# georghess/neurad-studio

Hardware: NVIDIA H100
Metric: rays/sec (camera+lidar) (higher is better)
Workload: dtype f32

## Files before the change

### neurad-studio_b200/csrc/b200nerf.cu

```cuda
#include <cuda_runtime.h>

#include <cstdio>
#include <cstring>
#include <new>
#include <string>
#include <vector>

#include "../../include/b200nerf.h"
#include "nff_device.h"
#include "nff_lane.h"
#include "rgb_decoder.cuh"
#include "modules.cuh"
#include "lidar_eval.cuh"
#include "lidar_loss.cuh"
#include "image_metrics.cuh"
#include "camera_rays.h"
#include "lidar_sim.cuh"

using namespace nff;

static thread_local std::string g_err;
static int fail(int code, const std::string& msg) {
  g_err = msg;
  return code;
// ... 197 lines not shown
    int64_t patch;
    if (it < full_rounds) {
      patch = (it * gridDim.x + blockIdx.x) * kPPU + warp;
    } else {
      patch = p0 + warp + (it - full_rounds) * kPPU;
      if (patch >= p1) break;
    }
    int64_t ray;
    const bool active = lane_patch_ray(P, patch, lane_, &ray);
    const LaneRay R = lane_ray_setup<ACTORS, EDIT>(P, sc, tid, ray);
    float* col = active ? handoff + ray : sc.bins2 + tid;
    sample_ray_lane<LAYOUT, ACTORS, TRACED>(P, sc, R, tid, ray, active, col, active ? P.n_rays : (int64_t)kLaneThreads,
                                            shared_edges ? e0_tab : nullptr);
  }
}
template <int LAYOUT>
static auto sample_lane_kernel(bool actors, bool traced, bool edit) {
  if (edit) return traced ? nff_sample_lane_kernel<LAYOUT, true, true, true> : nff_sample_lane_kernel<LAYOUT, true, false, true>;
  return traced ? nff_sample_lane_kernel<LAYOUT, true, true, false>
         : actors ? nff_sample_lane_kernel<LAYOUT, true, false, false>
                  : nff_sample_lane_kernel<LAYOUT, false, false, false>;
}

template <int LAYOUT, bool EDIT>
__global__ void __launch_bounds__(kLaneThreads, kLaneCtasPerSm) nff_shade_lane_kernel(const __grid_constant__ RenderParams P,
                                                                                      float* __restrict__ scratch,
                                                                                      const float* __restrict__ handoff) {
  extern __shared__ __align__(128) unsigned char smem_shade[];
  LaneTcShared* tcs = reinterpret_cast<LaneTcShared*>(smem_shade);
  const int tid = threadIdx.x, warp = __shfl_sync(0xffffffffu, (int)(threadIdx.x >> 5), 0), group = warp >> 2;
  lane_tc_stage_weights(*tcs, P.main_mlp_nn, tid, kLaneThreads);
  tc::fence_async_smem();
  __syncthreads();
  MlpLaneTc mlp;
  mlp.t = tcs;
  mlp.panel_ = reinterpret_cast<float*>(smem_shade + kLaneTcBytes);
  mlp.status = P.status;
  mlp.bar_id = 1 + group;
  const LaneScratch sc = lane_scratch_of(scratch, blockIdx.x);
  mlp.sh_tcnn = LAYOUT;
  constexpr int kPPU = kLaneThreads / 32;
  const int64_t n_patches = lane_patches(P);
  const int64_t full_rounds = n_patches / kPPU / gridDim.x;
  const int64_t r0 = full_rounds * gridDim.x * kPPU;
  const int64_t rest_groups = (n_patches - r0 + 3) / 4;
  const int64_t g0 = rest_groups * blockIdx.x / gridDim.x, g1 = rest_groups * (blockIdx.x + 1) / gridDim.x;
  for (int64_t it = 0;; ++it) {
    int64_t patch;
    if (it < full_rounds) {
      patch = (it * gridDim.x + blockIdx.x) * kPPU + warp;
    } else {
      const int64_t gu = g0 + group + (it - full_rounds) * (kLaneThreads / 128);
      if (gu >= g1) break;
      patch = r0 + gu * 4 + (warp & 3);
    }
    int64_t ray;
    const bool active = lane_patch_ray(P, patch, tid & 31, &ray);
    const LaneRay R = lane_ray_setup<true, EDIT>(P, sc, tid, ray);
    shade_ray_lane<MlpLaneTc, LAYOUT>(P, sc, R, mlp, tid, ray, active, handoff + ray, P.n_rays);
  }
}

template <bool EDIT>
__global__ void __launch_bounds__(kLaneThreads, kLaneCtasPerSm) nff_render_lane_kernel(const __grid_constant__ RenderParams P,
                                                                          float* __restrict__ scratch) {
  extern __shared__ __align__(128) unsigned char smem_lane[];
  LaneTcShared* tcs = reinterpret_cast<LaneTcShared*>(smem_lane);
  const int tid = threadIdx.x, warp = __shfl_sync(0xffffffffu, (int)(threadIdx.x >> 5), 0), group = warp >> 2;
  lane_tc_stage_weights(*tcs, P.main_mlp_nn, tid, kLaneThreads);
  tc::fence_async_smem();
  __syncthreads();
  MlpLaneTc mlp;
  mlp.t = tcs;
  mlp.panel_ = reinterpret_cast<float*>(smem_lane + kLaneTcBytes);
  mlp.status = P.status;
  mlp.bar_id = 1 + group;
  const LaneScratch sc = lane_scratch_of(scratch, blockIdx.x);
  for (int64_t unit = blockIdx.x; unit < lane_units(P); unit += gridDim.x) {
    int64_t ray;
    const bool active = lane_unit_ray(P, unit, tid, &ray);
    render_ray_lane<MlpLaneTc, 0, EDIT>(P, sc, mlp, tid, ray, active);
  }
}
// ... 653 lines not shown
  int n = 0;
  CUDA_TRY(cudaGetDeviceCount(&n));
  REQUIRE(device_ordinal >= 0 && device_ordinal < n, "device ordinal out of range");
  DeviceGuard g(device_ordinal);
  cudaDeviceProp prop;
  CUDA_TRY(cudaGetDeviceProperties(&prop, device_ordinal));
  if (prop.major != 9 || prop.minor != 0)
    return fail(B200NERF_ERR_UNSUPPORTED, "libb200nerf is built for sm_90a only (found sm_" +
                                              std::to_string(prop.major) + std::to_string(prop.minor) + ")");
  b200nerf_ctx* c = new (std::nothrow) b200nerf_ctx();
  REQUIRE(c != nullptr, "out of host memory");
  c->device = device_ordinal;
  c->sm_count = prop.multiProcessorCount;
  CUDA_TRY(cudaFuncSetAttribute(nff_render_kernel<kRenderWarps>, cudaFuncAttributeMaxDynamicSharedMemorySize,
                                (int)((kMainMlpFloats * 4 + 15) / 16 * 16 + kRenderWarps * sizeof(WarpShared))));
  CUDA_TRY(cudaFuncSetAttribute(nff_render_tc_kernel<kRenderWarps>, cudaFuncAttributeMaxDynamicSharedMemorySize,
                                (int)(tc_smem_bytes(kRenderWarps * 32) + kRenderWarps * sizeof(WarpSharedTc))));
  CUDA_TRY(cudaMalloc((void**)&c->d_status, sizeof(int)));
  CUDA_TRY(cudaMemset(c->d_status, 0, sizeof(int)));
  for (auto k : {nff_render_lane_kernel<false>, nff_render_lane_kernel<true>})
    CUDA_TRY(cudaFuncSetAttribute(k, cudaFuncAttributeMaxDynamicSharedMemorySize, (int)lane_tc_smem_bytes()));
  c->lane_ctas = c->sm_count * (kLaneCtasPerSm > NFF_SAMPLE_CTAS ? kLaneCtasPerSm : NFF_SAMPLE_CTAS);
  CUDA_TRY(cudaMalloc((void**)&c->d_lane_scratch, sizeof(float) * lane_scratch_floats_per_cta() * c->lane_ctas));
  for (auto k : {nff_shade_lane_kernel<0, false>, nff_shade_lane_kernel<1, false>, nff_shade_lane_kernel<0, true>,
                 nff_shade_lane_kernel<1, true>})
    CUDA_TRY(cudaFuncSetAttribute(k, cudaFuncAttributeMaxDynamicSharedMemorySize, (int)lane_tc_smem_bytes()));
  for (int i = 0; i < 8; ++i) {
    CUDA_TRY(cudaFuncSetAttribute(sample_lane_kernel<0>(i & 1, i & 2, i & 4), cudaFuncAttributePreferredSharedMemoryCarveout, 0));
    CUDA_TRY(cudaFuncSetAttribute(sample_lane_kernel<1>(i & 1, i & 2, i & 4), cudaFuncAttributePreferredSharedMemoryCarveout, 0));
  }
  CUDA_TRY(cudaMalloc((void**)&c->d_minmax, 2 * sizeof(unsigned)));
  c->handoff_rays = (int64_t)1 << 21;
  CUDA_TRY(cudaMalloc((void**)&c->d_handoff, sizeof(float) * (kS2 + 1) * c->handoff_rays));
  CUDA_TRY(cudaMalloc((void**)&c->d_grad_actor_ptrs, sizeof(float*) * kModMaxActors));
  CUDA_TRY(cudaMalloc((void**)&c->d_im_minmax, sizeof(float) * 4 * kImMaxBlocks));
  CUDA_TRY(cudaMalloc((void**)&c->d_im_sums, sizeof(double) * (kImMaxBlocks + kSsimMaxTiles)));
  *out = c;
  return 0;
}

int b200nerf_destroy(b200nerf_ctx* c) {
  if (!c) return 0;
  DeviceGuard g(c->device);
  for (int i = 0; i < 3; ++i) {
    cudaFree((void*)c->d_actor_tables[i]);
    cudaFree(c->d_decoder[i]);
  }
  cudaFree(c->d_main_mlp);
  cudaFree(c->d_main_mlp_nn);
// ... 356 lines not shown
    int64_t slice = c->handoff_rays;
    if (rays->image_width > 0) {
      const int64_t band = (int64_t)rays->image_width * (kLaneThreads / 32);
      REQUIRE(band <= slice, "image_width too large for the two-stage renderer");
      slice = slice / band * band;
    }
    const int fdim = kNff + c->app.dim;
    for (int64_t start = 0; start < n_rays; start += slice) {
      const int64_t cnt = n_rays - start < slice ? n_rays - start : slice;
      RenderParams Q = P;
      Q.n_rays = cnt;
      offset_rays(Q, start, fdim);
      int64_t need = (cnt + kLaneThreads - 1) / kLaneThreads;
      if (rays->image_width > 0) {
        const int64_t W = rays->image_width, H = (cnt + W - 1) / W;
        need = ((W + 31) / 32) * ((H + kLaneThreads / 32 - 1) / (kLaneThreads / 32));
      }
      const int64_t max_a = (int64_t)c->sm_count * NFF_SAMPLE_CTAS, max_b = (int64_t)c->sm_count * kLaneCtasPerSm;
      const int64_t patches = rays->image_width > 0 ? need * (kLaneThreads / 32) : (cnt + 31) / 32, groups = (patches + 3) / 4;
      const int64_t grid_a = patches < max_a ? patches : max_a, grid_b = groups < max_b ? groups : max_b;
      const bool actors = c->actors.n_actors > 0;
      if (c->layout == 1) {
        sample_lane_kernel<1>(actors, traced, edit)<<<(int)grid_a, kLaneThreads, 0, st>>>(Q, c->d_lane_scratch, c->d_handoff);
        (edit ? nff_shade_lane_kernel<1, true> : nff_shade_lane_kernel<1, false>)<<<(int)grid_b, kLaneThreads, smem, st>>>(
            Q, c->d_lane_scratch, c->d_handoff);
      } else {
        sample_lane_kernel<0>(actors, traced, edit)<<<(int)grid_a, kLaneThreads, 0, st>>>(Q, c->d_lane_scratch, c->d_handoff);
        (edit ? nff_shade_lane_kernel<0, true> : nff_shade_lane_kernel<0, false>)<<<(int)grid_b, kLaneThreads, smem, st>>>(
            Q, c->d_lane_scratch, c->d_handoff);
      }
    }
  } else if (c->mlp_mode == 2) {
    const size_t smem = lane_tc_smem_bytes();
    int64_t need = (n_rays + kLaneThreads - 1) / kLaneThreads;
    if (rays->image_width > 0) {
      const int64_t W = rays->image_width, H = (n_rays + W - 1) / W;
      need = ((W + 31) / 32) * ((H + kLaneThreads / 32 - 1) / (kLaneThreads / 32));
    }
    int lane_blocks = (int)(need < c->lane_ctas ? need : c->lane_ctas);
    (edit ? nff_render_lane_kernel<true> : nff_render_lane_kernel<false>)<<<lane_blocks, kLaneThreads, smem, st>>>(
        P, c->d_lane_scratch);
  } else if (c->mlp_mode == 1) {
    const size_t smem = tc_smem_bytes(WARPS * 32) + WARPS * sizeof(WarpSharedTc);
    nff_render_tc_kernel<WARPS><<<blocks, WARPS * 32, smem, st>>>(P);
  } else {
    const size_t smem = (kMainMlpFloats * 4 + 15) / 16 * 16 + WARPS * sizeof(WarpShared);
    nff_render_kernel<WARPS><<<blocks, WARPS * 32, smem, st>>>(P);
  }
  CUDA_TRY(cudaGetLastError());
  if (out->intensity || out->ray_drop_logit) {
    int fdim = kNff + c->app.dim;
    lidar_decode_kernel<<<(unsigned)((n_rays + 127) / 128), 128, 0, st>>>(c->d_lidar_mlp, out->features, fdim, n_rays,
// ... 1207 lines not shown
```

### neurad-studio_b200/csrc/nff_device.h

```cpp
#pragma once
#include "nff_params.h"
#include "simt.h"

#ifndef NFF_G_PROP
#define NFF_G_PROP 1
#endif
#ifndef NFF_G_ACT
#define NFF_G_ACT 2
#endif
#ifndef NFF_ILP
#define NFF_ILP 2
#endif
#ifndef NFF_F4_UNROLL
#define NFF_F4_UNROLL 2
#endif
#ifndef NFF_FAST_RCP
#define NFF_FAST_RCP 1
#endif
#ifndef NFF_PARITY_STD
#define NFF_PARITY_STD 0
#endif
#ifndef NFF_PARITY_LERP
#define NFF_PARITY_LERP 0
#endif
// ... 314 lines not shown
#pragma unroll
  for (int d = 0; d < D; ++d) w = fmul(w, (c & (1 << d)) ? frac[d] : fsub(1.0f, frac[d]));
  return w;
}
template <int D>
NFF_D float tcnn_encode_f1_dot(const Grid& gr, int L, const float* x, float std, const float* NFF_RESTRICT dec) {
  float acc = 0.0f;
#pragma unroll 1
  for (int l = 0; l < L; ++l) {
    uint32_t idx[1 << D];
    float frac[D];
    tcnn_corners<D>(gr, l, x, idx, frac);
    float f[1 << D];
#pragma unroll
    for (int c = 0; c < (1 << D); ++c) f[c] = ldg(gr.table + idx[c]);
    float v = 0.0f;
#pragma unroll
    for (int c = 0; c < (1 << D); ++c) v = fmaf(tcnn_corner_weight<D>(c, frac), f[c], v);
    acc = fmaf(fmul(v, level_weight(gr.res[l], std)), ldg(dec + l), acc);
  }
  return acc;
}
template <int D>
NFF_D void tcnn_encode_f4(const Grid& gr, int L, const float* x, float std, float* out, int stride) {
#pragma unroll 1
  for (int l = 0; l < L; ++l) {
    uint32_t idx[1 << D];
    float frac[D];
    tcnn_corners<D>(gr, l, x, idx, frac);
    const float4* t4 = reinterpret_cast<const float4*>(gr.table);
    float4 v[1 << D];
#pragma unroll
    for (int c = 0; c < (1 << D); ++c) v[c] = ldg(t4 + idx[c]);
    float a0 = 0.0f, a1 = 0.0f, a2 = 0.0f, a3 = 0.0f;
#pragma unroll
    for (int c = 0; c < (1 << D); ++c) {
      const float w = tcnn_corner_weight<D>(c, frac);
      a0 = fmaf(w, v[c].x, a0);
      a1 = fmaf(w, v[c].y, a1);
      a2 = fmaf(w, v[c].z, a2);
      a3 = fmaf(w, v[c].w, a3);
    }
    const float lw = level_weight(gr.res[l], std);
    out[(4 * l + 0) * stride] = fmul(a0, lw);
    out[(4 * l + 1) * stride] = fmul(a1, lw);
    out[(4 * l + 2) * stride] = fmul(a2, lw);
    out[(4 * l + 3) * stride] = fmul(a3, lw);
  }
}
NFF_D void sh4_tcnn(float dx, float dy, float dz, float* c) {
  const float x = fsub(fmul(fmul(fadd(dx, 1.0f), 0.5f), 2.0f), 1.0f), y = fsub(fmul(fmul(fadd(dy, 1.0f), 0.5f), 2.0f), 1.0f),
              z = fsub(fmul(fmul(fadd(dz, 1.0f), 0.5f), 2.0f), 1.0f);
  const float xy = x * y, xz = x * z, yz = y * z, x2 = x * x, y2 = y * y, z2 = z * z;
  c[0] = 0.28209479177387814f;
  c[1] = -0.48860251190291987f * y;
  c[2] = 0.48860251190291987f * z;
  c[3] = -0.48860251190291987f * x;
  c[4] = 1.0925484305920792f * xy;
  c[5] = -1.0925484305920792f * yz;
  c[6] = 0.94617469575755997f * z2 - 0.31539156525251999f;
  c[7] = -1.0925484305920792f * xz;
  c[8] = 0.54627421529603959f * x2 - 0.54627421529603959f * y2;
  c[9] = 0.59004358992664352f * y * (-3.0f * x2 + y2);
  c[10] = 2.8906114426405538f * xy * z;
  c[11] = 0.45704579946446572f * y * (1.0f - 5.0f * z2);
  c[12] = 0.3731763325901154f * z * (5.0f * z2 - 3.0f);
// ... 589 lines not shown
```

### neurad-studio_b200/csrc/nff_lane.h

```cpp
#pragma once
#include "nff_device.h"

namespace nff {

#ifndef NFF_LANE_THREADS
#define NFF_LANE_THREADS 512
#endif
#ifndef NFF_F4_WEIGHTS
#define NFF_F4_WEIGHTS 0
#endif
constexpr int kLaneThreads = NFF_LANE_THREADS;
constexpr int kLaneCtasPerSm = 512 / kLaneThreads;
constexpr int kCandFloats = 16;
constexpr int kLaneMaxCand = 32;

struct LaneScratch {
  float* w;
  float* bins1;
  float* bins2;
  float* cand;
};
NFF_HD size_t lane_scratch_floats_per_cta() {
  return (size_t)kLaneThreads * (kS0 + (kS1 + 1) + (kS2 + 1) + kLaneMaxCand * kCandFloats);
}
// ... 107 lines not shown
  float acc;
  if (a >= 0) {
    Gauss ga = {pb[0], pb[1], pb[2], g.std};
    ga = contract(ga, fg.actor_scale);
    if (LAYOUT == 1) {
      const float x4[4] = {ga.x, ga.y, ga.z, fdiv((float)a, fg.n_actors_f)};
      acc = tcnn_encode_f1_dot<4>(fg.act, 4, x4, ga.std, fg.decoder);
    } else {
      acc = encode_f1_dot<4, NFF_G_ACT>(fg.actor_tables[a], fg.act, ga, fg.decoder);
    }
  } else {
    Gauss gs = contract(g, fg.static_scale);
    if (LAYOUT == 1) {
      const float x3[3] = {gs.x, gs.y, gs.z};
      acc = tcnn_encode_f1_dot<3>(fg.stat, 6, x3, gs.std, fg.decoder);
    } else {
      acc = encode_f1_dot<6, NFF_G_PROP>(fg.stat.table, fg.stat, gs, fg.decoder);
    }
  }
  *actor_id = a;
  return expf(acc);
}

NFF_D void encode_f4_col(const float* NFF_RESTRICT table, const Grid& gr, int L, Gauss g, float* x , int pitch) {
  const uint32_t maskb = gr.mask << 4;
#pragma unroll 2
  for (int l = 0; l < L; ++l) {
    const float res = gr.res[l];
    const CellB<4> c = grid_cell_b<4>(g.x, g.y, g.z, res);
    uint32_t r[8];
    cell_offsets_b<4>(c, maskb, r);
    const char* base = level_base(table, l, gr.T, 16);
    float4 v[8];
#pragma unroll
    for (int k = 0; k < 8; ++k) v[k] = ldg_at<float4>(base, r[k]);
    float w = level_weight(res, g.std);
    const float ix = 1.0f - c.ox, iy = 1.0f - c.oy, iz = 1.0f - c.oz;
#if NFF_F4_WEIGHTS
    const float z1 = c.oz * w, z0 = iz * w;
    const float y1z1 = c.oy * z1, y0z1 = iy * z1, y1z0 = c.oy * z0, y0z0 = iy * z0;
    const float wk[8] = {c.ox * y1z1, c.ox * y0z1, ix * y0z1, ix * y1z1, c.ox * y1z0, c.ox * y0z0, ix * y0z0, ix * y1z0};
    float a0 = wk[0] * v[0].x, a1 = wk[0] * v[0].y, a2 = wk[0] * v[0].z, a3 = wk[0] * v[0].w;
#pragma unroll
    for (int k = 1; k < 8; ++k) {
      a0 = fmaf(wk[k], v[k].x, a0);
      a1 = fmaf(wk[k], v[k].y, a1);
      a2 = fmaf(wk[k], v[k].z, a2);
      a3 = fmaf(wk[k], v[k].w, a3);
    }
    x[(4 * l + 0) * pitch] = a0;
    x[(4 * l + 1) * pitch] = a1;
    x[(4 * l + 2) * pitch] = a2;
    x[(4 * l + 3) * pitch] = a3;
#else
    float f[8];
#pragma unroll
    for (int k = 0; k < 8; ++k) f[k] = v[k].x;
    x[(4 * l + 0) * pitch] = fmul(trilerp_b<4>(f, c, ix, iy, iz), w);
#pragma unroll
// ... 70 lines not shown
      c_km1 = c_k;
      if (k <= S) {
        const float wk = w_next;
        w_next = sc.w[(size_t)(k < S ? k : S - 1) * kLaneThreads + tid];
        run += (double)fdiv(fadd(wk, pad_each), tot);
        c_k = fminf(1.0f, (float)run);
      }
    }
    const int above = k > S ? S : k;
    const float b0 = edge(k - 1), b1 = edge(above);
    float t = nan_to_num(fdiv(fsub(u, c_km1), fsub(k > S ? c_km1 : c_k, c_km1)));
    t = fminf(fmaxf(t, 0.0f), 1.0f);
    const float nb = fadd(b0, fmul(t, fsub(b1, b0)));
    io.bins_out[(size_t)i * io.bins_stride] = nb;
    if (TRACED && io.tr_inds) io.tr_inds[ray * (S_new + 1) + i] = k;
    if (TRACED && io.tr_bins_s) io.tr_bins_s[ray * (S_new + 1) + i] = nb;
    if (TRACED && io.tr_bins_e) io.tr_bins_e[ray * (S_new + 1) + i] = to_euclid(nb, s_near, s_far, sp);
  }
  return depth_acc;
}

struct MlpLaneFfma {
  static constexpr int kPitch = kLaneThreads;
  const float* w;
  float* panel_;
  int sh_tcnn = 0;
  NFF_D float* panel() const { return panel_; }
  NFF_D void run(const float* x, const float dir[3], float& sdf, float* feat, int ) const {
    float h[kHidden], go[kNff + 1], in2[kNff + kSh], h2[kHidden];
    dense<kGeoIn, kHidden, kHidden, true>(w + kOffGeoW0, w + kOffGeoB0, x, h);
    dense<kHidden, kNff + 1, kGeoOutP, false>(w + kOffGeoW1, w + kOffGeoB1, h, go);
    sdf = go[0];
#pragma unroll
    for (int i = 0; i < kNff; ++i) in2[i] = go[i + 1];
    if (sh_tcnn) sh4_tcnn(dir[0], dir[1], dir[2], in2 + kNff); else sh4(dir[0], dir[1], dir[2], in2 + kNff);
    dense<kNff + kSh, kHidden, kHidden, true>(w + kOffFeatW0, w + kOffFeatB0, in2, h);
    dense<kHidden, kHidden, kHidden, true>(w + kOffFeatW1, w + kOffFeatB1, h, h2);
    dense<kHidden, kNff, kNff, false>(w + kOffFeatW2, w + kOffFeatB2, h2, h);
#pragma unroll
    for (int i = 0; i < kNff; ++i) feat[i] = in2[i] + h[i];
  }
};

#if defined(__CUDACC__)
constexpr int kLanePanelPitch = kLaneThreads + 4;
constexpr int kLanePanelRows = kGeoIn + kSh + 1;
constexpr int kLaneTcA = 6;
constexpr float kLaneTcAScale = 64.0f, kLaneTcAUnscale = 1.0f / 64.0f;
constexpr float kLaneTcOverflow = 65520.0f;
constexpr int kLaneTcRangeStatus = 4;
struct LaneTcShared {
  __half b[2 * 32 * (32 + 32 + 48 + 32 + 32)];
  float bias[kTcLayers][32];
  float up[kTcLayers], down[kTcLayers];
  float w_sdf[32];
  float b_sdf;
  unsigned wmax[kTcLayers];
};
constexpr int kLaneTcBytes = (sizeof(LaneTcShared) + 127) / 128 * 128;
constexpr size_t lane_tc_smem_bytes() { return (size_t)kLaneTcBytes + sizeof(float) * kLanePanelRows * kLanePanelPitch; }

NFF_D void lane_tc_stage_weights(LaneTcShared& t, const float* NFF_RESTRICT nn, int tid, int nthreads) {
  if (tid < kTcLayers) t.wmax[tid] = 0u;
  __syncthreads();
#pragma unroll
  for (int l = 0; l < kTcLayers; ++l) {
    unsigned m = 0u;
    for (int i = tid; i < 32 * tc_layer_k(l); i += nthreads) m = max(m, __float_as_uint(fabsf(nn[tc_layer_w(l) + i])));
    m = __reduce_max_sync(0xffffffffu, m);
    if ((tid & 31) == 0 && m) atomicMax(&t.wmax[l], m);
  }
  __syncthreads();
#pragma unroll
  for (int l = 0; l < kTcLayers; ++l) {
    int E;
    frexpf(__uint_as_float(t.wmax[l]), &E);
    const int e = min(max(15 - E, -60), 60);
    const float up = __int_as_float((127 + e) << 23), down = __int_as_float((127 - e) << 23);
    const int K = tc_layer_k(l);
    __half* hi = t.b + tc_layer_off(l);
    tc::stage_b_tile_f16(hi, hi + 32 * K, nn + tc_layer_w(l), K, up, tid, nthreads);
    for (int i = tid; i < 32; i += nthreads) t.bias[l][i] = nn[tc_layer_b(l) + i] * up * kLaneTcAScale;
    if (tid == 0) t.up[l] = up, t.down[l] = down;
  }
  for (int i = tid; i < 32; i += nthreads) t.w_sdf[i] = nn[kNnGeoW1 + i];
  if (tid == 0) t.b_sdf = nn[kNnGeoB1];
}

struct MlpLaneTc {
  static constexpr int kPitch = kLanePanelPitch;
  const LaneTcShared* t;
  float* panel_;
  int* status;
  int bar_id;
  int sh_tcnn = 0;
  NFF_D float* panel() const { return panel_; }
  NFF_D void group_sync() const { asm volatile("bar.sync %0, 128;" ::"r"(bar_id) : "memory"); }

  NFF_D static uint32_t b_desc_lo() {
    extern __shared__ __align__(128) unsigned char nff_lane_smem[];
    return tc::smem_desc_lo(tc::smem_u32(nff_lane_smem + offsetof(LaneTcShared, b)), 128u);
  }

  template <int KS, int K, int OFF>
  NFF_D void half_mma(float* acc, const float* a) const {
    uint32_t ah[4 * KS], al[4 * KS];
    float amax = 0.0f;
#pragma unroll
    for (int i = 0; i < 4 * KS; ++i) {
      amax = fmaxf(amax, fmaxf(fabsf(a[2 * i]), fabsf(a[2 * i + 1])));
      tc::f16x2_split(a[2 * i], a[2 * i + 1], ah[i], al[i]);
    }
    if (amax >= kLaneTcOverflow && status) atomicExch(status, kLaneTcRangeStatus);
    constexpr uint32_t sbo = (uint32_t)(K / 8) * 128u;
    constexpr uint32_t hi_off = (uint32_t)OFF * 2u / 16u, lo_off = (uint32_t)(OFF + 32 * K) * 2u / 16u;
    const uint32_t b_desc = b_desc_lo();
    tc::wg_fence();
#pragma unroll
    for (int ks = 0; ks < KS; ++ks) {
      const uint32_t adv = (uint32_t)(ks * 2 * 128) / 16u;
      const uint64_t dh = tc::smem_desc_of(b_desc + hi_off + adv, sbo), dl = tc::smem_desc_of(b_desc + lo_off + adv, sbo);
      tc::wgmma_f16_m64n32(acc, ah + 4 * ks, dh);
      tc::wgmma_f16_m64n32(acc, al + 4 * ks, dh);
      tc::wgmma_f16_m64n32(acc, ah + 4 * ks, dl);
    }
    tc::wg_commit();
    tc::wg_wait<0>();
    tc::reg_fence(acc, 16);
#pragma unroll
    for (int i = 0; i < 4 * KS; ++i) asm volatile("" : "+r"(ah[i]), "+r"(al[i])::"memory");
  }
  NFF_D static void load_a(float* a, const float* p, int q, int ks0, int n) {
#pragma unroll
    for (int i = 0; i < n; ++i) {
      const float* r = p + (16 * (ks0 + i) + 2 * q) * kPitch;
      a[8 * i + 0] = r[0] * kLaneTcAScale;
      a[8 * i + 1] = r[kPitch] * kLaneTcAScale;
      a[8 * i + 2] = r[8] * kLaneTcAScale;
      a[8 * i + 3] = r[kPitch + 8] * kLaneTcAScale;
      a[8 * i + 4] = r[8 * kPitch] * kLaneTcAScale;
      a[8 * i + 5] = r[9 * kPitch] * kLaneTcAScale;
      a[8 * i + 6] = r[8 * kPitch + 8] * kLaneTcAScale;
      a[8 * i + 7] = r[9 * kPitch + 8] * kLaneTcAScale;
    }
  }
  NFF_D static void bias_init(float* acc, const float* bias, int q) {
#pragma unroll
    for (int j = 0; j < 4; ++j) {
      const float2 b = *reinterpret_cast<const float2*>(bias + 8 * j + 2 * q);
      acc[4 * j + 0] = acc[4 * j + 2] = b.x;
      acc[4 * j + 1] = acc[4 * j + 3] = b.y;
    }
  }
  NFF_D static void unscale(float* acc, float down) {
#pragma unroll
    for (int i = 0; i < 16; ++i) acc[i] *= down;
  }
  NFF_D static void relu(float* acc) {
#pragma unroll
    for (int i = 0; i < 16; ++i) acc[i] = fmaxf(acc[i], 0.0f);
  }

  NFF_D void run(const float* , const float dir[3], float& sdf, float* feat, int tid) {
    float* col = panel_ + tid;
    {
      float shv[kSh];
      if (sh_tcnn) sh4_tcnn(dir[0], dir[1], dir[2], shv); else sh4(dir[0], dir[1], dir[2], shv);
#pragma unroll
      for (int i = 0; i < kSh; ++i) col[(kGeoIn + i) * kPitch] = shv[i];
    }
    group_sync();
    const int ln = tid & 31, q = ln & 3;
    float* const fr = panel_ + (tid & ~127) + 16 * ((tid >> 5) & 3) + (ln >> 2);
#pragma unroll 1
    for (int h = 0; h < 2; ++h) {
      float* const p = fr + 64 * h;
      float a[24], acc[16];
      load_a(a, p, q, 0, 2);
      bias_init(acc, t->bias[0], q);
      half_mma<2, 32, tc_layer_off(0)>(acc, a);
      unscale(acc, t->down[0]);
      relu(acc);
      float s0 = 0.0f, s1 = 0.0f;
#pragma unroll
      for (int j = 0; j < 4; ++j) {
        const float2 w = *reinterpret_cast<const float2*>(t->w_sdf + 8 * j + 2 * q);
        s0 = fmaf(acc[4 * j + 0], w.x, fmaf(acc[4 * j + 1], w.y, s0));
        s1 = fmaf(acc[4 * j + 2], w.x, fmaf(acc[4 * j + 3], w.y, s1));
      }
      s0 += __shfl_xor_sync(0xffffffffu, s0, 1);
      s1 += __shfl_xor_sync(0xffffffffu, s1, 1);
      s0 += __shfl_xor_sync(0xffffffffu, s0, 2);
      s1 += __shfl_xor_sync(0xffffffffu, s1, 2);
      if (q == 0) {
        p[(kGeoIn + kSh) * kPitch] = s0 * kLaneTcAUnscale + t->b_sdf;
        p[(kGeoIn + kSh) * kPitch + 8] = s1 * kLaneTcAUnscale + t->b_sdf;
      }
#pragma unroll
      for (int i = 0; i < 16; ++i) a[i] = acc[i];
      bias_init(acc, t->bias[1], q);
      half_mma<2, 32, tc_layer_off(1)>(acc, a);
      unscale(acc, t->down[1]);
      __syncwarp();
#pragma unroll
      for (int j = 0; j < 4; ++j) {
        float* r = p + (8 * j + 2 * q) * kPitch;
        r[0] = acc[4 * j + 0], r[kPitch] = acc[4 * j + 1], r[8] = acc[4 * j + 2], r[kPitch + 8] = acc[4 * j + 3];
      }
#pragma unroll
      for (int i = 0; i < 16; ++i) a[i] = acc[i];
      load_a(a + 16, p, q, 2, 1);
      bias_init(acc, t->bias[2], q);
      half_mma<3, 48, tc_layer_off(2)>(acc, a);
      unscale(acc, t->down[2]);
      relu(acc);
#pragma unroll
      for (int i = 0; i < 16; ++i) a[i] = acc[i];
      bias_init(acc, t->bias[3], q);
      half_mma<2, 32, tc_layer_off(3)>(acc, a);
      unscale(acc, t->down[3]);
      relu(acc);
#pragma unroll
      for (int i = 0; i < 16; ++i) a[i] = acc[i];
      bias_init(acc, t->bias[4], q);
      const float up4 = t->up[4], out4 = t->down[4] * kLaneTcAUnscale;
#pragma unroll
      for (int j = 0; j < 4; ++j) {
        const float* r = p + (8 * j + 2 * q) * kPitch;
        acc[4 * j + 0] += r[0] * up4, acc[4 * j + 1] += r[kPitch] * up4;
        acc[4 * j + 2] += r[8] * up4, acc[4 * j + 3] += r[kPitch + 8] * up4;
      }
      half_mma<2, 32, tc_layer_off(4)>(acc, a);
#pragma unroll
      for (int j = 0; j < 4; ++j) {
        float* r = p + (8 * j + 2 * q) * kPitch;
        r[0] = acc[4 * j + 0] * out4, r[kPitch] = acc[4 * j + 1] * out4;
        r[8] = acc[4 * j + 2] * out4, r[kPitch + 8] = acc[4 * j + 3] * out4;
      }
    }
    group_sync();
#pragma unroll
    for (int i = 0; i < kNff; ++i) feat[i] = col[i * kPitch];
    sdf = col[(kGeoIn + kSh) * kPitch];
  }
};
#endif

struct LaneRay {
  float o[3], d[3];
  float area, time, s_near, s_far;
  int n_cand;
};
constexpr float kDefaultNear = 0.0f, kDefaultFar = 1.0e6f;
NFF_D void lane_spacing_bounds(const Sampling& sp, float near_, float far_, float* s_near, float* s_far) {
  *s_near = spacing_fn(near_, sp);
  *s_far = spacing_fn(fminf(far_, sp.sky_distance), sp);
}
NFF_D float lane_round0_edge(const Sampling& sp, int i) {
  float s_near, s_far;
  lane_spacing_bounds(sp, kDefaultNear, kDefaultFar, &s_near, &s_far);
// ... 28 lines not shown
  const Sampling& sp = P.samp;
#pragma unroll 1
  for (int rd = 0; rd < 2; ++rd) {
    LaneRoundIO io{};
    io.S = rd == 0 ? kS0 : kS1;
    io.S_new = rd == 0 ? kS1 : kS2;
    io.u_tab = rd == 0 ? sp.u1 : sp.u2;
    io.bins_out = rd == 0 ? sc.bins1 + tid : bins2;
    io.bins_stride = rd == 0 ? (int64_t)kLaneThreads : bins2_stride;
    if (TRACED) {
      io.tr_w = !active ? nullptr : rd == 0 ? P.trace.prop_weights_0 : P.trace.prop_weights_1;
      io.tr_aid = !active ? nullptr : rd == 0 ? P.trace.actor_id_0 : P.trace.actor_id_1;
      io.tr_bins_s = !active ? nullptr : rd == 0 ? P.trace.bins_s_1 : P.trace.bins_s_2;
      io.tr_bins_e = !active ? nullptr : rd == 0 ? P.trace.bins_e_1 : P.trace.bins_e_2;
      io.tr_inds = !active ? nullptr : rd == 0 ? P.trace.inds_1 : P.trace.inds_2;
    }
    const float prop_depth = lane_proposal_round<LAYOUT, ACTORS, TRACED>(
        P, P.fields[sp.field_of_round[rd]], sc, tid, R.n_cand, io, rd == 0 ? nullptr : sc.bins1 + tid,
        rd == 0 ? e0_tab : nullptr, R.o, R.d, R.area, R.s_near, R.s_far, ray);
    if (active) (rd == 0 ? P.out.prop_depth_0 : P.out.prop_depth_1)[ray] = prop_depth;
  }
}

template <class Mlp, int LAYOUT = 0>
NFF_D void shade_ray_lane(const RenderParams& P, const LaneScratch& sc, const LaneRay& R, Mlp& mlp, int tid, int64_t ray,
                          bool active, const float* bins2, int64_t bins2_stride) {
  const Sampling& sp = P.samp;
  const float* o = R.o;
  const float* d = R.d;
  const float area = R.area, time = R.time, s_near = R.s_near, s_far = R.s_far;
  const int n_cand = R.n_cand;

  const FieldGrids& fm = P.fields[B200NERF_FIELD_MAIN];
  float fsum[kNff];
#pragma unroll
  for (int i = 0; i < kNff; ++i) fsum[i] = 0.0f;
  double T_d = 1.0;
  float acc = 0.0f, depth = 0.0f;
  float e_prev = to_euclid(bins2[0], s_near, s_far, sp);
#pragma unroll 1
  for (int s = 0; s < kS2; ++s) {
    const float e0 = e_prev;
    float e1 = to_euclid(bins2[(size_t)(s + 1) * bins2_stride], s_near, s_far, sp);
    e_prev = e1;
    if (s == kS2 - 1) e1 = fadd(e1, fsub(sp.sky_distance, e1));
    Gauss g = sample_gaussian(o, d, area, e0, e1);
    float* col = mlp.panel() + tid;
    float dir[3] = {d[0], d[1], d[2]};
    int aid = -1;
    {
      float pb[3], M[12];
      aid = n_cand > 0 ? lane_actor_of_sample(sc, tid, n_cand, g, pb, M) : -1;
      if (aid >= 0) {
        Gauss ga = {pb[0], pb[1], pb[2], g.std};
        ga = contract(ga, fm.actor_scale);
#pragma unroll
        for (int i = 16; i < 32; ++i) col[i * Mlp::kPitch] = 0.0f;
        if (LAYOUT == 1) {
          const float x4[4] = {ga.x, ga.y, ga.z, fdiv((float)aid, fm.n_actors_f)};
          tcnn_encode_f4<4>(fm.act, 4, x4, ga.std, col, Mlp::kPitch);
        } else {
          encode_f4_col(fm.actor_tables[aid], fm.act, 4, ga, col, Mlp::kPitch);
        }
        float q0 = fadd(fadd(fmul(M[0], d[0]), fmul(M[1], d[1])), fmul(M[2], d[2]));
        float q1 = fadd(fadd(fmul(M[4], d[0]), fmul(M[5], d[1])), fmul(M[6], d[2]));
        float q2 = fadd(fadd(fmul(M[8], d[0]), fmul(M[9], d[1])), fmul(M[10], d[2]));
        float n = fadd(fsqrt(fadd(fadd(fmul(q0, q0), fmul(q1, q1)), fmul(q2, q2))), 1.0e-7f);
        dir[0] = fdiv(q0, n); dir[1] = fdiv(q1, n); dir[2] = fdiv(q2, n);
      } else {
        Gauss gs = contract(g, fm.static_scale);
        if (LAYOUT == 1) {
          const float x3[3] = {gs.x, gs.y, gs.z};
          tcnn_encode_f4<3>(fm.stat, 8, x3, gs.std, col, Mlp::kPitch);
        } else {
          encode_f4_col(fm.stat.table, fm.stat, 8, gs, col, Mlp::kPitch);
        }
      }
    }
    float x[kGeoIn];
#pragma unroll
    for (int i = 0; i < kGeoIn; ++i) x[i] = col[i * Mlp::kPitch];
    float sdf, feat[kNff];
    mlp.run(x, dir, sdf, feat, tid);
    const float alpha = frcp(fadd(1.0f, expf(fmul(sdf, P.beta))));
    float w = fmul(alpha, (float)T_d);
    T_d *= (double)fsub(1.0f, alpha);
    acc = fadd(acc, w);
    if (s < kS2 - 1) depth = fadd(depth, fmul(w, fmul(fadd(e0, e1), 0.5f)));
    if (s == kS2 - 1) w = fadd(fadd(w, 1.0f), -acc);
#pragma unroll
    for (int i = 0; i < kNff; ++i) fsum[i] = fmaf(feat[i], w, fsum[i]);
    if (active) {
      if (P.trace.sdf) P.trace.sdf[ray * kS2 + s] = sdf;
      if (P.trace.alpha) P.trace.alpha[ray * kS2 + s] = alpha;
      if (P.trace.weights) P.trace.weights[ray * kS2 + s] = w;
      if (P.trace.actor_id_main) P.trace.actor_id_main[ray * kS2 + s] = aid;
      if (P.trace.field_feature) {
#pragma unroll
        for (int i = 0; i < kNff; ++i) P.trace.field_feature[(ray * kS2 + s) * kNff + i] = feat[i];
      }
    }
  }
  const int fdim = P.nff_dim + P.app.dim;
  float app[kApp];
#pragma unroll
  for (int i = 0; i < kApp; ++i) app[i] = 0.0f;
// ... 86 lines not shown
```

### neurad-studio_b200/csrc/tc_mlp.cuh

```cuda
#pragma once
#include <cuda_fp16.h>
#include <cuda_runtime.h>
#include <stdint.h>

namespace tc {

__device__ __forceinline__ uint32_t smem_u32(const void* p) { return (uint32_t)__cvta_generic_to_shared(p); }

__device__ __forceinline__ void fence_async_smem() { asm volatile("fence.proxy.async.shared::cta;" ::: "memory"); }
__device__ __forceinline__ void wg_fence() { asm volatile("wgmma.fence.sync.aligned;" ::: "memory"); }
__device__ __forceinline__ void wg_commit() { asm volatile("wgmma.commit_group.sync.aligned;" ::: "memory"); }
template <int N>
__device__ __forceinline__ void wg_wait() { asm volatile("wgmma.wait_group.sync.aligned %0;" ::"n"(N) : "memory"); }
__device__ __forceinline__ void reg_fence(float* d, int n) {
  for (int i = 0; i < n; ++i) asm volatile("" : "+f"(d[i])::"memory");
}

__device__ __forceinline__ void mbar_init(uint64_t* bar, uint32_t count) {
  asm volatile("mbarrier.init.shared::cta.b64 [%0], %1;" ::"r"(smem_u32(bar)), "r"(count) : "memory");
  asm volatile("fence.mbarrier_init.release.cluster;" ::: "memory");
}
__device__ __forceinline__ bool mbar_wait(uint64_t* bar, uint32_t parity) {
  const uint32_t addr = smem_u32(bar);
  for (int it = 0; it < (1 << 20); ++it) {
// ... 56 lines not shown
  asm volatile("{\n\t.reg .pred p;\n\tsetp.ne.b32 p, %34, 0;\n\twgmma.mma_async.sync.aligned.m64n64k16.f32.bf16.bf16 "
               "{%0, %1, %2, %3, %4, %5, %6, %7, %8, %9, %10, %11, %12, %13, %14, %15, %16, %17, %18, %19, %20, %21, %22, %23, %24, %25, %26, %27, %28, %29, %30, %31}, %32, %33, p, 1, 1, 0, 0;\n\t}"
               : TC_D32(0)
               : "l"(a_desc), "l"(b_desc), "r"(1));
}
__device__ __forceinline__ void wgmma_bf16_m64n96(float* d, uint64_t a_desc, uint64_t b_desc) {
  asm volatile("{\n\t.reg .pred p;\n\tsetp.ne.b32 p, %50, 0;\n\twgmma.mma_async.sync.aligned.m64n96k16.f32.bf16.bf16 "
               "{%0, %1, %2, %3, %4, %5, %6, %7, %8, %9, %10, %11, %12, %13, %14, %15, %16, %17, %18, %19, %20, %21, %22, %23, %24, %25, %26, %27, %28, %29, %30, %31, %32, %33, %34, %35, %36, %37, %38, %39, %40, %41, %42, %43, %44, %45, %46, %47}, %48, %49, p, 1, 1, 0, 0;\n\t}"
               : TC_D32(0), TC_D16(32)
               : "l"(a_desc), "l"(b_desc), "r"(1));
}
__device__ __forceinline__ void wgmma_bf16_m64n128(float* d, uint64_t a_desc, uint64_t b_desc) {
  asm volatile("{\n\t.reg .pred p;\n\tsetp.ne.b32 p, %66, 0;\n\twgmma.mma_async.sync.aligned.m64n128k16.f32.bf16.bf16 "
               "{%0, %1, %2, %3, %4, %5, %6, %7, %8, %9, %10, %11, %12, %13, %14, %15, %16, %17, %18, %19, %20, %21, %22, %23, %24, %25, %26, %27, %28, %29, %30, %31, %32, %33, %34, %35, %36, %37, %38, %39, %40, %41, %42, %43, %44, %45, %46, %47, %48, %49, %50, %51, %52, %53, %54, %55, %56, %57, %58, %59, %60, %61, %62, %63}, %64, %65, p, 1, 1, 0, 0;\n\t}"
               : TC_D32(0), TC_D32(32)
               : "l"(a_desc), "l"(b_desc), "r"(1));
}
__device__ __forceinline__ void wgmma_f16_m64n32(float* d, const uint32_t* a, uint64_t b_desc) {
  asm volatile("{\n\t.reg .pred p;\n\tsetp.ne.b32 p, %21, 0;\n\twgmma.mma_async.sync.aligned.m64n32k16.f32.f16.f16 "
               "{%0, %1, %2, %3, %4, %5, %6, %7, %8, %9, %10, %11, %12, %13, %14, %15}, {%16, %17, %18, %19}, %20, p, 1, 1, 0;\n\t}"
               : TC_D16(0)
               : "r"(a[0]), "r"(a[1]), "r"(a[2]), "r"(a[3]), "l"(b_desc), "r"(1));
}
template <int N>
__device__ __forceinline__ void wgmma_tf32(float* d, const uint32_t* a, uint64_t b_desc) {
  static_assert(N == 16 || N == 32 || N == 48 || N == 64, "tf32 tile widths");
  if constexpr (N == 16) wgmma_tf32_m64n16(d, a, b_desc);
  else if constexpr (N == 32) wgmma_tf32_m64n32(d, a, b_desc);
  else if constexpr (N == 48) wgmma_tf32_m64n48(d, a, b_desc);
  else wgmma_tf32_m64n64(d, a, b_desc);
}

__host__ __device__ constexpr uint32_t b_tile_floats(int n_pad, int k_pad) { return (uint32_t)(n_pad * k_pad); }
__device__ __forceinline__ uint32_t b_elem_offset(int n, int k, int k_pad) {
  return (uint32_t)((n >> 3) * (k_pad >> 2) * 32 + (k >> 2) * 32 + (n & 7) * 4 + (k & 3));
}
__device__ __forceinline__ float tf32_hi(float x) { return __uint_as_float(__float_as_uint(x) & 0xffffe000u); }

__device__ __forceinline__ void stage_b_tile(float* hi, float* lo, const float* __restrict__ w, int n_real, int k_real, int n_pad,
                                             int k_pad, int tid, int nthreads) {
  for (int i = tid; i < n_pad * k_pad; i += nthreads) {
    int n = i / k_pad, k = i % k_pad;
    float v = (n < n_real && k < k_real) ? w[n * k_real + k] : 0.0f;
    float h = tf32_hi(v);
    uint32_t off = b_elem_offset(n, k, k_pad);
    hi[off] = h;
// ... 120 lines not shown
```

Measured before the change: 91.04 million.

## Fold activation scaling into encoders and bias into epilogue; specialize shade kernel on actors

Adds an ACTORS template parameter to the shade lane kernel so scenes without actors skip actor lookup and compute the SH direction encoding once per ray rather than per sample. The TC MLP no longer multiplies A-operands by the scale when loading. Instead the encoders write pre-scaled features, the first wgmma zero-initializes the accumulator, and bias plus unscale are fused into one FMA epilogue. Overflow detection now uses half2 max on the split values, and the up factor is dropped. These changes remove per-sample multiplies and register traffic, but they alter the numerics of range checking and bias handling.

```diff
diff --git a/neurad-studio_b200/csrc/b200nerf.cu b/neurad-studio_b200/csrc/b200nerf.cu
--- a/neurad-studio_b200/csrc/b200nerf.cu
+++ b/neurad-studio_b200/csrc/b200nerf.cu
@@ -243,7 +243,7 @@
                   : nff_sample_lane_kernel<LAYOUT, false, false, false>;
 }
 
-template <int LAYOUT, bool EDIT>
+template <int LAYOUT, bool ACTORS, bool EDIT>
 __global__ void __launch_bounds__(kLaneThreads, kLaneCtasPerSm) nff_shade_lane_kernel(const __grid_constant__ RenderParams P,
                                                                                       float* __restrict__ scratch,
                                                                                       const float* __restrict__ handoff) {
@@ -277,9 +277,15 @@
     }
     int64_t ray;
     const bool active = lane_patch_ray(P, patch, tid & 31, &ray);
-    const LaneRay R = lane_ray_setup<true, EDIT>(P, sc, tid, ray);
-    shade_ray_lane<MlpLaneTc, LAYOUT>(P, sc, R, mlp, tid, ray, active, handoff + ray, P.n_rays);
-  }
+    const LaneRay R = lane_ray_setup<ACTORS, EDIT>(P, sc, tid, ray);
+    shade_ray_lane<MlpLaneTc, LAYOUT, ACTORS>(P, sc, R, mlp, tid, ray, active, handoff + ray, P.n_rays);
+  }
+}
+template <int LAYOUT>
+static auto shade_lane_kernel(bool actors, bool edit) {
+  return edit ? nff_shade_lane_kernel<LAYOUT, true, true>
+         : actors ? nff_shade_lane_kernel<LAYOUT, true, false>
+                  : nff_shade_lane_kernel<LAYOUT, false, false>;
 }
 
 template <bool EDIT>
@@ -979,9 +985,9 @@
     CUDA_TRY(cudaFuncSetAttribute(k, cudaFuncAttributeMaxDynamicSharedMemorySize, (int)lane_tc_smem_bytes()));
   c->lane_ctas = c->sm_count * (kLaneCtasPerSm > NFF_SAMPLE_CTAS ? kLaneCtasPerSm : NFF_SAMPLE_CTAS);
   CUDA_TRY(cudaMalloc((void**)&c->d_lane_scratch, sizeof(float) * lane_scratch_floats_per_cta() * c->lane_ctas));
-  for (auto k : {nff_shade_lane_kernel<0, false>, nff_shade_lane_kernel<1, false>, nff_shade_lane_kernel<0, true>,
-                 nff_shade_lane_kernel<1, true>})
-    CUDA_TRY(cudaFuncSetAttribute(k, cudaFuncAttributeMaxDynamicSharedMemorySize, (int)lane_tc_smem_bytes()));
+  for (int i = 0; i < 4; ++i)
+    for (auto k : {shade_lane_kernel<0>(i & 1, i & 2), shade_lane_kernel<1>(i & 1, i & 2)})
+      CUDA_TRY(cudaFuncSetAttribute(k, cudaFuncAttributeMaxDynamicSharedMemorySize, (int)lane_tc_smem_bytes()));
   for (int i = 0; i < 8; ++i) {
     CUDA_TRY(cudaFuncSetAttribute(sample_lane_kernel<0>(i & 1, i & 2, i & 4), cudaFuncAttributePreferredSharedMemoryCarveout, 0));
     CUDA_TRY(cudaFuncSetAttribute(sample_lane_kernel<1>(i & 1, i & 2, i & 4), cudaFuncAttributePreferredSharedMemoryCarveout, 0));
@@ -1384,12 +1390,10 @@
       const bool actors = c->actors.n_actors > 0;
       if (c->layout == 1) {
         sample_lane_kernel<1>(actors, traced, edit)<<<(int)grid_a, kLaneThreads, 0, st>>>(Q, c->d_lane_scratch, c->d_handoff);
-        (edit ? nff_shade_lane_kernel<1, true> : nff_shade_lane_kernel<1, false>)<<<(int)grid_b, kLaneThreads, smem, st>>>(
-            Q, c->d_lane_scratch, c->d_handoff);
+        shade_lane_kernel<1>(actors, edit)<<<(int)grid_b, kLaneThreads, smem, st>>>(Q, c->d_lane_scratch, c->d_handoff);
       } else {
         sample_lane_kernel<0>(actors, traced, edit)<<<(int)grid_a, kLaneThreads, 0, st>>>(Q, c->d_lane_scratch, c->d_handoff);
-        (edit ? nff_shade_lane_kernel<0, true> : nff_shade_lane_kernel<0, false>)<<<(int)grid_b, kLaneThreads, smem, st>>>(
-            Q, c->d_lane_scratch, c->d_handoff);
+        shade_lane_kernel<0>(actors, edit)<<<(int)grid_b, kLaneThreads, smem, st>>>(Q, c->d_lane_scratch, c->d_handoff);
       }
     }
   } else if (c->mlp_mode == 2) {
diff --git a/neurad-studio_b200/csrc/nff_device.h b/neurad-studio_b200/csrc/nff_device.h
--- a/neurad-studio_b200/csrc/nff_device.h
+++ b/neurad-studio_b200/csrc/nff_device.h
@@ -360,7 +360,7 @@
   return acc;
 }
 template <int D>
-NFF_D void tcnn_encode_f4(const Grid& gr, int L, const float* x, float std, float* out, int stride) {
+NFF_D void tcnn_encode_f4(const Grid& gr, int L, const float* x, float std, float* out, int stride, float scale) {
 #pragma unroll 1
   for (int l = 0; l < L; ++l) {
     uint32_t idx[1 << D];
@@ -379,7 +379,7 @@
       a2 = fmaf(w, v[c].z, a2);
       a3 = fmaf(w, v[c].w, a3);
     }
-    const float lw = level_weight(gr.res[l], std);
+    const float lw = fmul(level_weight(gr.res[l], std), scale);
     out[(4 * l + 0) * stride] = fmul(a0, lw);
     out[(4 * l + 1) * stride] = fmul(a1, lw);
     out[(4 * l + 2) * stride] = fmul(a2, lw);
diff --git a/neurad-studio_b200/csrc/nff_lane.h b/neurad-studio_b200/csrc/nff_lane.h
--- a/neurad-studio_b200/csrc/nff_lane.h
+++ b/neurad-studio_b200/csrc/nff_lane.h
@@ -153,7 +153,8 @@
   return expf(acc);
 }
 
-NFF_D void encode_f4_col(const float* NFF_RESTRICT table, const Grid& gr, int L, Gauss g, float* x , int pitch) {
+NFF_D void encode_f4_col(const float* NFF_RESTRICT table, const Grid& gr, int L, Gauss g, float* x , int pitch,
+                         float scale) {
   const uint32_t maskb = gr.mask << 4;
 #pragma unroll 2
   for (int l = 0; l < L; ++l) {
@@ -165,7 +166,7 @@
     float4 v[8];
 #pragma unroll
     for (int k = 0; k < 8; ++k) v[k] = ldg_at<float4>(base, r[k]);
-    float w = level_weight(res, g.std);
+    const float w = fmul(level_weight(res, g.std), scale);
     const float ix = 1.0f - c.ox, iy = 1.0f - c.oy, iz = 1.0f - c.oz;
 #if NFF_F4_WEIGHTS
     const float z1 = c.oz * w, z0 = iz * w;
@@ -282,18 +283,24 @@
 
 struct MlpLaneFfma {
   static constexpr int kPitch = kLaneThreads;
+  static constexpr float kAScale = 1.0f;
   const float* w;
   float* panel_;
   int sh_tcnn = 0;
+  float sh_[kSh] = {};
   NFF_D float* panel() const { return panel_; }
-  NFF_D void run(const float* x, const float dir[3], float& sdf, float* feat, int ) const {
+  NFF_D void set_dir(const float dir[3], int ) {
+    if (sh_tcnn) sh4_tcnn(dir[0], dir[1], dir[2], sh_); else sh4(dir[0], dir[1], dir[2], sh_);
+  }
+  NFF_D void run(const float* x, float& sdf, float* feat, int ) const {
     float h[kHidden], go[kNff + 1], in2[kNff + kSh], h2[kHidden];
     dense<kGeoIn, kHidden, kHidden, true>(w + kOffGeoW0, w + kOffGeoB0, x, h);
     dense<kHidden, kNff + 1, kGeoOutP, false>(w + kOffGeoW1, w + kOffGeoB1, h, go);
     sdf = go[0];
 #pragma unroll
     for (int i = 0; i < kNff; ++i) in2[i] = go[i + 1];
-    if (sh_tcnn) sh4_tcnn(dir[0], dir[1], dir[2], in2 + kNff); else sh4(dir[0], dir[1], dir[2], in2 + kNff);
+#pragma unroll
+    for (int i = 0; i < kSh; ++i) in2[kNff + i] = sh_[i];
     dense<kNff + kSh, kHidden, kHidden, true>(w + kOffFeatW0, w + kOffFeatB0, in2, h);
     dense<kHidden, kHidden, kHidden, true>(w + kOffFeatW1, w + kOffFeatB1, h, h2);
     dense<kHidden, kNff, kNff, false>(w + kOffFeatW2, w + kOffFeatB2, h2, h);
@@ -311,9 +318,9 @@
 constexpr int kLaneTcRangeStatus = 4;
 struct LaneTcShared {
   __half b[2 * 32 * (32 + 32 + 48 + 32 + 32)];
-  float bias[kTcLayers][32];
-  float up[kTcLayers], down[kTcLayers];
-  float w_sdf[32];
+  alignas(8) float bias[kTcLayers][32];
+  float down[kTcLayers];
+  alignas(8) float w_sdf[32];
   float b_sdf;
   unsigned wmax[kTcLayers];
 };
@@ -340,8 +347,8 @@
     const int K = tc_layer_k(l);
     __half* hi = t.b + tc_layer_off(l);
     tc::stage_b_tile_f16(hi, hi + 32 * K, nn + tc_layer_w(l), K, up, tid, nthreads);
-    for (int i = tid; i < 32; i += nthreads) t.bias[l][i] = nn[tc_layer_b(l) + i] * up * kLaneTcAScale;
-    if (tid == 0) t.up[l] = up, t.down[l] = down;
+    for (int i = tid; i < 32; i += nthreads) t.bias[l][i] = nn[tc_layer_b(l) + i] * (l < kTcLayers - 1 ? kLaneTcAScale : 1.0f);
+    if (tid == 0) t.down[l] = down;
   }
   for (int i = tid; i < 32; i += nthreads) t.w_sdf[i] = nn[kNnGeoW1 + i];
   if (tid == 0) t.b_sdf = nn[kNnGeoB1];
@@ -349,6 +356,7 @@
 
 struct MlpLaneTc {
   static constexpr int kPitch = kLanePanelPitch;
+  static constexpr float kAScale = kLaneTcAScale;
   const LaneTcShared* t;
   float* panel_;
   int* status;
@@ -365,13 +373,14 @@
   template <int KS, int K, int OFF>
   NFF_D void half_mma(float* acc, const float* a) const {
     uint32_t ah[4 * KS], al[4 * KS];
-    float amax = 0.0f;
+    __half2 amax = __float2half2_rn(0.0f);
 #pragma unroll
     for (int i = 0; i < 4 * KS; ++i) {
-      amax = fmaxf(amax, fmaxf(fabsf(a[2 * i]), fabsf(a[2 * i + 1])));
       tc::f16x2_split(a[2 * i], a[2 * i + 1], ah[i], al[i]);
-    }
-    if (amax >= kLaneTcOverflow && status) atomicExch(status, kLaneTcRangeStatus);
+      amax = __hmax2(amax, __habs2(*reinterpret_cast<const __half2*>(&ah[i])));
+    }
+    if (__hge2_mask(amax, __half2half2(__ushort_as_half((unsigned short)0x7c00u))) != 0u && status)
+      atomicExch(status, kLaneTcRangeStatus);
     constexpr uint32_t sbo = (uint32_t)(K / 8) * 128u;
     constexpr uint32_t hi_off = (uint32_t)OFF * 2u / 16u, lo_off = (uint32_t)(OFF + 32 * K) * 2u / 16u;
     const uint32_t b_desc = b_desc_lo();
@@ -380,7 +389,8 @@
     for (int ks = 0; ks < KS; ++ks) {
       const uint32_t adv = (uint32_t)(ks * 2 * 128) / 16u;
       const uint64_t dh = tc::smem_desc_of(b_desc + hi_off + adv, sbo), dl = tc::smem_desc_of(b_desc + lo_off + adv, sbo);
-      tc::wgmma_f16_m64n32(acc, ah + 4 * ks, dh);
+      if (ks == 0) tc::wgmma_f16_m64n32_zero(acc, ah, dh);
+      else tc::wgmma_f16_m64n32(acc, ah + 4 * ks, dh);
       tc::wgmma_f16_m64n32(acc, al + 4 * ks, dh);
       tc::wgmma_f16_m64n32(acc, ah + 4 * ks, dl);
     }
@@ -394,41 +404,41 @@
 #pragma unroll
     for (int i = 0; i < n; ++i) {
       const float* r = p + (16 * (ks0 + i) + 2 * q) * kPitch;
-      a[8 * i + 0] = r[0] * kLaneTcAScale;
-      a[8 * i + 1] = r[kPitch] * kLaneTcAScale;
-      a[8 * i + 2] = r[8] * kLaneTcAScale;
-      a[8 * i + 3] = r[kPitch + 8] * kLaneTcAScale;
-      a[8 * i + 4] = r[8 * kPitch] * kLaneTcAScale;
-      a[8 * i + 5] = r[9 * kPitch] * kLaneTcAScale;
-      a[8 * i + 6] = r[8 * kPitch + 8] * kLaneTcAScale;
-      a[8 * i + 7] = r[9 * kPitch + 8] * kLaneTcAScale;
-    }
-  }
-  NFF_D static void bias_init(float* acc, const float* bias, int q) {
+      a[8 * i + 0] = r[0];
+      a[8 * i + 1] = r[kPitch];
+      a[8 * i + 2] = r[8];
+      a[8 * i + 3] = r[kPitch + 8];
+      a[8 * i + 4] = r[8 * kPitch];
+      a[8 * i + 5] = r[9 * kPitch];
+      a[8 * i + 6] = r[8 * kPitch + 8];
+      a[8 * i + 7] = r[9 * kPitch + 8];
+    }
+  }
+  NFF_D static void rescale_bias(float* acc, float down, const float* bias, int q) {
 #pragma unroll
     for (int j = 0; j < 4; ++j) {
       const float2 b = *reinterpret_cast<const float2*>(bias + 8 * j + 2 * q);
-      acc[4 * j + 0] = acc[4 * j + 2] = b.x;
-      acc[4 * j + 1] = acc[4 * j + 3] = b.y;
-    }
-  }
-  NFF_D static void unscale(float* acc, float down) {
-#pragma unroll
-    for (int i = 0; i < 16; ++i) acc[i] *= down;
+      acc[4 * j + 0] = fmaf(acc[4 * j + 0], down, b.x);
+      acc[4 * j + 1] = fmaf(acc[4 * j + 1], down, b.y);
+      acc[4 * j + 2] = fmaf(acc[4 * j + 2], down, b.x);
+      acc[4 * j + 3] = fmaf(acc[4 * j + 3], down, b.y);
+    }
   }
   NFF_D static void relu(float* acc) {
 #pragma unroll
     for (int i = 0; i < 16; ++i) acc[i] = fmaxf(acc[i], 0.0f);
   }
 
-  NFF_D void run(const float* , const float dir[3], float& sdf, float* feat, int tid) {
+  NFF_D void set_dir(const float dir[3], int tid) const {
+    float shv[kSh];
+    if (sh_tcnn) sh4_tcnn(dir[0], dir[1], dir[2], shv); else sh4(dir[0], dir[1], dir[2], shv);
     float* col = panel_ + tid;
-    {
-      float shv[kSh];
-      if (sh_tcnn) sh4_tcnn(dir[0], dir[1], dir[2], shv); else sh4(dir[0], dir[1], dir[2], shv);
-#pragma unroll
-      for (int i = 0; i < kSh; ++i) col[(kGeoIn + i) * kPitch] = shv[i];
-    }
+#pragma unroll
+    for (int i = 0; i < kSh; ++i) col[(kGeoIn + i) * kPitch] = shv[i] * kLaneTcAScale;
+  }
+
+  NFF_D void run(const float* , float& sdf, float* feat, int tid) {
+    float* col = panel_ + tid;
     group_sync();
     const int ln = tid & 31, q = ln & 3;
     float* const fr = panel_ + (tid & ~127) + 16 * ((tid >> 5) & 3) + (ln >> 2);
@@ -437,9 +447,8 @@
       float* const p = fr + 64 * h;
       float a[24], acc[16];
       load_a(a, p, q, 0, 2);
-      bias_init(acc, t->bias[0], q);
       half_mma<2, 32, tc_layer_off(0)>(acc, a);
-      unscale(acc, t->down[0]);
+      rescale_bias(acc, t->down[0], t->bias[0], q);
       relu(acc);
       float s0 = 0.0f, s1 = 0.0f;
 #pragma unroll
@@ -458,9 +467,8 @@
       }
 #pragma unroll
       for (int i = 0; i < 16; ++i) a[i] = acc[i];
-      bias_init(acc, t->bias[1], q);
       half_mma<2, 32, tc_layer_off(1)>(acc, a);
-      unscale(acc, t->down[1]);
+      rescale_bias(acc, t->down[1], t->bias[1], q);
       __syncwarp();
 #pragma unroll
       for (int j = 0; j < 4; ++j) {
@@ -470,32 +478,26 @@
 #pragma unroll
       for (int i = 0; i < 16; ++i) a[i] = acc[i];
       load_a(a + 16, p, q, 2, 1);
-      bias_init(acc, t->bias[2], q);
       half_mma<3, 48, tc_layer_off(2)>(acc, a);
-      unscale(acc, t->down[2]);
+      rescale_bias(acc, t->down[2], t->bias[2], q);
       relu(acc);
 #pragma unroll
       for (int i = 0; i < 16; ++i) a[i] = acc[i];
-      bias_init(acc, t->bias[3], q);
       half_mma<2, 32, tc_layer_off(3)>(acc, a);
-      unscale(acc, t->down[3]);
+      rescale_bias(acc, t->down[3], t->bias[3], q);
       relu(acc);
 #pragma unroll
       for (int i = 0; i < 16; ++i) a[i] = acc[i];
-      bias_init(acc, t->bias[4], q);
-      const float up4 = t->up[4], out4 = t->down[4] * kLaneTcAUnscale;
-#pragma unroll
-      for (int j = 0; j < 4; ++j) {
-        const float* r = p + (8 * j + 2 * q) * kPitch;
-        acc[4 * j + 0] += r[0] * up4, acc[4 * j + 1] += r[kPitch] * up4;
-        acc[4 * j + 2] += r[8] * up4, acc[4 * j + 3] += r[kPitch + 8] * up4;
-      }
       half_mma<2, 32, tc_layer_off(4)>(acc, a);
+      const float out4 = t->down[4] * kLaneTcAUnscale;
 #pragma unroll
       for (int j = 0; j < 4; ++j) {
         float* r = p + (8 * j + 2 * q) * kPitch;
-        r[0] = acc[4 * j + 0] * out4, r[kPitch] = acc[4 * j + 1] * out4;
-        r[8] = acc[4 * j + 2] * out4, r[kPitch + 8] = acc[4 * j + 3] * out4;
+        const float2 b = *reinterpret_cast<const float2*>(t->bias[4] + 8 * j + 2 * q);
+        r[0] = fmaf(acc[4 * j + 0], out4, fmaf(r[0], kLaneTcAUnscale, b.x));
+        r[kPitch] = fmaf(acc[4 * j + 1], out4, fmaf(r[kPitch], kLaneTcAUnscale, b.y));
+        r[8] = fmaf(acc[4 * j + 2], out4, fmaf(r[8], kLaneTcAUnscale, b.x));
+        r[kPitch + 8] = fmaf(acc[4 * j + 3], out4, fmaf(r[kPitch + 8], kLaneTcAUnscale, b.y));
       }
     }
     group_sync();
@@ -570,7 +572,7 @@
   }
 }
 
-template <class Mlp, int LAYOUT = 0>
+template <class Mlp, int LAYOUT = 0, bool ACTORS = true>
 NFF_D void shade_ray_lane(const RenderParams& P, const LaneScratch& sc, const LaneRay& R, Mlp& mlp, int tid, int64_t ray,
                           bool active, const float* bins2, int64_t bins2_stride) {
   const Sampling& sp = P.samp;
@@ -586,6 +588,7 @@
   double T_d = 1.0;
   float acc = 0.0f, depth = 0.0f;
   float e_prev = to_euclid(bins2[0], s_near, s_far, sp);
+  if (!ACTORS) mlp.set_dir(d, tid);
 #pragma unroll 1
   for (int s = 0; s < kS2; ++s) {
     const float e0 = e_prev;
@@ -594,11 +597,11 @@
     if (s == kS2 - 1) e1 = fadd(e1, fsub(sp.sky_distance, e1));
     Gauss g = sample_gaussian(o, d, area, e0, e1);
     float* col = mlp.panel() + tid;
-    float dir[3] = {d[0], d[1], d[2]};
     int aid = -1;
     {
+      float dir[3] = {d[0], d[1], d[2]};
       float pb[3], M[12];
-      aid = n_cand > 0 ? lane_actor_of_sample(sc, tid, n_cand, g, pb, M) : -1;
+      if (ACTORS && n_cand > 0) aid = lane_actor_of_sample(sc, tid, n_cand, g, pb, M);
       if (aid >= 0) {
         Gauss ga = {pb[0], pb[1], pb[2], g.std};
         ga = contract(ga, fm.actor_scale);
@@ -606,9 +609,9 @@
         for (int i = 16; i < 32; ++i) col[i * Mlp::kPitch] = 0.0f;
         if (LAYOUT == 1) {
           const float x4[4] = {ga.x, ga.y, ga.z, fdiv((float)aid, fm.n_actors_f)};
-          tcnn_encode_f4<4>(fm.act, 4, x4, ga.std, col, Mlp::kPitch);
+          tcnn_encode_f4<4>(fm.act, 4, x4, ga.std, col, Mlp::kPitch, Mlp::kAScale);
         } else {
-          encode_f4_col(fm.actor_tables[aid], fm.act, 4, ga, col, Mlp::kPitch);
+          encode_f4_col(fm.actor_tables[aid], fm.act, 4, ga, col, Mlp::kPitch, Mlp::kAScale);
         }
         float q0 = fadd(fadd(fmul(M[0], d[0]), fmul(M[1], d[1])), fmul(M[2], d[2]));
         float q1 = fadd(fadd(fmul(M[4], d[0]), fmul(M[5], d[1])), fmul(M[6], d[2]));
@@ -619,17 +622,18 @@
         Gauss gs = contract(g, fm.static_scale);
         if (LAYOUT == 1) {
           const float x3[3] = {gs.x, gs.y, gs.z};
-          tcnn_encode_f4<3>(fm.stat, 8, x3, gs.std, col, Mlp::kPitch);
+          tcnn_encode_f4<3>(fm.stat, 8, x3, gs.std, col, Mlp::kPitch, Mlp::kAScale);
         } else {
-          encode_f4_col(fm.stat.table, fm.stat, 8, gs, col, Mlp::kPitch);
+          encode_f4_col(fm.stat.table, fm.stat, 8, gs, col, Mlp::kPitch, Mlp::kAScale);
         }
       }
+      if (ACTORS) mlp.set_dir(dir, tid);
     }
     float x[kGeoIn];
 #pragma unroll
     for (int i = 0; i < kGeoIn; ++i) x[i] = col[i * Mlp::kPitch];
     float sdf, feat[kNff];
-    mlp.run(x, dir, sdf, feat, tid);
+    mlp.run(x, sdf, feat, tid);
     const float alpha = frcp(fadd(1.0f, expf(fmul(sdf, P.beta))));
     float w = fmul(alpha, (float)T_d);
     T_d *= (double)fsub(1.0f, alpha);
diff --git a/neurad-studio_b200/csrc/tc_mlp.cuh b/neurad-studio_b200/csrc/tc_mlp.cuh
--- a/neurad-studio_b200/csrc/tc_mlp.cuh
+++ b/neurad-studio_b200/csrc/tc_mlp.cuh
@@ -102,6 +102,13 @@
                : TC_D16(0)
                : "r"(a[0]), "r"(a[1]), "r"(a[2]), "r"(a[3]), "l"(b_desc), "r"(1));
 }
+__device__ __forceinline__ void wgmma_f16_m64n32_zero(float* d, const uint32_t* a, uint64_t b_desc) {
+  asm volatile("{\n\t.reg .pred p;\n\tsetp.ne.b32 p, %21, 0;\n\twgmma.mma_async.sync.aligned.m64n32k16.f32.f16.f16 "
+               "{%0, %1, %2, %3, %4, %5, %6, %7, %8, %9, %10, %11, %12, %13, %14, %15}, {%16, %17, %18, %19}, %20, p, 1, 1, 0;\n\t}"
+               : "=f"(d[0]), "=f"(d[1]), "=f"(d[2]), "=f"(d[3]), "=f"(d[4]), "=f"(d[5]), "=f"(d[6]), "=f"(d[7]),
+                 "=f"(d[8]), "=f"(d[9]), "=f"(d[10]), "=f"(d[11]), "=f"(d[12]), "=f"(d[13]), "=f"(d[14]), "=f"(d[15])
+               : "r"(a[0]), "r"(a[1]), "r"(a[2]), "r"(a[3]), "l"(b_desc), "r"(0));
+}
 template <int N>
 __device__ __forceinline__ void wgmma_tf32(float* d, const uint32_t* a, uint64_t b_desc) {
   static_assert(N == 16 || N == 32 || N == 48 || N == 64, "tf32 tile widths");
```

After: 93.78 million (median of 6 runs). +3.0%, better.
